# inferflow/inferflow

Hardware: AMD Instinct MI355X
Metric: decode tokens/sec, Llama-2-7B Q4 batch=1 greedy (whole job) (higher is better)
Workload: dtype i8 (Q8 activations x Q4_B32T1A weights, i32 dot, f32 scale, f16 I/O); 1 GPU; llama2_7b decode, Q4_B32T1A weights + F16 lm_head, F16 KV cache, batch 1 greedy, 16-token prompt, context 21..1851; parallelism=single, weights_bytes=4309647360

## Files before the change

include/inferflow_amd.h:

```cpp
#ifndef INFERFLOW_AMD_H_
#define INFERFLOW_AMD_H_

#include <stddef.h>
#include <stdint.h>

#ifdef __cplusplus
extern "C" {
#endif

typedef enum {
    IFA_F32 = 0, IFA_F16 = 1,
    IFA_Q8_B32T1 = 7, IFA_Q8_B32T2 = 8, IFA_Q6_B64T1 = 9, IFA_Q5_B64T1 = 10, IFA_Q5_B32T1 = 11,
    IFA_Q4_B16 = 12, IFA_Q4_B32T1A = 13, IFA_Q4_B32T1B = 14, IFA_Q4_B64T1 = 17, IFA_Q3H_B64T1 = 18,
    IFA_Q3_B32T1A = 19, IFA_Q3_B32T1B = 20, IFA_Q2_B32T1A = 21, IFA_Q2_B32T1B = 22
} ifa_dtype;

enum {
    IFA_OK = 0,
    IFA_ERR_ARG = -1,
    IFA_ERR_DTYPE = -2,
    IFA_ERR_HIP = -3,
    IFA_ERR_STATE = -4,
    IFA_ERR_NOMEM = -5
};
// ... 124 lines not shown
int ifa_model_create(const ifa_model_config *cfg, ifa_model **out);
int ifa_model_destroy(ifa_model *m);
int ifa_model_set_tensor(ifa_model *m, int layer, int tensor_id, int expert, int dtype,
                         const void *dev_src, size_t rows, size_t cols);
int ifa_model_set_tensor_f16(ifa_model *m, int layer, int tensor_id, int expert, int target_dtype,
                             const void *dev_src_f16, size_t rows, size_t cols);
int ifa_model_finalize(ifa_model *m);
int ifa_model_reset(ifa_model *m);
int ifa_model_kv_slots(ifa_model *m, int n_slots);
int ifa_model_select_kv(ifa_model *m, int slot);
int ifa_model_kv_copy(ifa_model *m, int src_slot, int dst_slot, int n_rows);
int ifa_model_kv_shift(ifa_model *m, int slot, int keep, int discard, int n_rows);
int ifa_kv_shift_rows(int kv_dtype, void *kcache, void *vcache, size_t kv_heads, size_t head_dim, int rope_order, int rope_cols,
                      const float *table_dev, size_t keep, size_t discard, size_t n_rows, ifa_stream stream);
int ifa_model_set_option(ifa_model *m, const char *name, int value);
int ifa_model_set_excluded_tokens(ifa_model *m, const int *ids_host, int n);
int ifa_model_perf_stat(ifa_model *m, int *keys_out, float *ms_out, int cap, int *n_out, int clear);
int ifa_model_fused_supported(ifa_model *m, char *why, size_t why_len);
int ifa_model_forward(ifa_model *m, const int *tokens_host, int n_tokens, int prefix_len,
                      void *logits_out_dev, int *next_token_host);
int ifa_model_decode(ifa_model *m, int first_token, int start_pos, int n_steps,
                     int *out_tokens_host, float *elapsed_ms);
int ifa_model_decode_prepare(ifa_model *m, int start_pos, int n_steps);
int ifa_model_decode_batch(ifa_model *m, int n, const int *tokens_host, const int *positions_host, const int *kv_slots_host,
                           int *next_tokens_host, void *logits_out_dev);
int ifa_model_decode_draft(ifa_model *m, int n, const int *tokens_host, int pos0, int *next_tokens_host, void *logits_out_dev);
int ifa_model_set_pool_excluded(ifa_model *m, const int *ids_host, int n);
int ifa_model_decode_pool(ifa_model *m, int token, int pos, int k, int *next_token_host,
                          int *pool_ids_host, unsigned short *pool_vals_host, int *pool_count_host);
int ifa_model_decode_batch_pool(ifa_model *m, int n, const int *tokens_host, const int *positions_host, const int *kv_slots_host,
                                int *next_tokens_host, int k, const int *rows_sel_host, int n_sel,
                                int *pool_ids_host, unsigned short *pool_vals_host, int *pool_counts_host);
int ifa_model_forward_pool(ifa_model *m, const int *tokens_host, int n_tokens, int prefix_len, void *logits_out_dev, int k,
                           int *next_token_host, int *pool_ids_host, unsigned short *pool_vals_host, int *pool_count_host);
int ifa_model_pool_lse(ifa_model *m, float *lse_host, int cap, int *n_out);
#define IFA_LOGIT_BIAS_MAX 1024
int ifa_model_logit_state_reset(ifa_model *m, int kv_slot, const int *prompt_host, int n_prompt, float rep, float freq, float pres,
                                const int *bias_ids_host, const float *bias_vals_host, int n_bias);
int ifa_model_logit_state_add(ifa_model *m, int n, const int *kv_slots_host, const int *tokens_host);
int ifa_model_pool_adjust(ifa_model *m, int n_sel, const int *state_slots_host);
int ifa_model_forward_score(ifa_model *m, const int *tokens_host, int n_tokens, int prefix_len, const int *targets_host,
                            float *lse_host, float *target_logit_host, int *next_token_host);
int ifa_model_get_buffer(ifa_model *m, const char *name, int layer, void **dptr, size_t *bytes);
void *ifa_model_stream(ifa_model *m);
int ifa_debug_alloc_fail_at(long long nth);
int ifa_debug_live_allocs(long long *count, long long *bytes);
// ... 59 lines not shown
```

inferflow_amd/_capi.py:

```python
import ctypes as C
import os

_HERE = os.path.dirname(os.path.abspath(__file__))
_LIB_PATH = os.environ.get("IFA_LIB") or os.path.join(_HERE, "lib", "libinferflow_amd.so")
_lib = None


class IfaError(RuntimeError):
    def __init__(self, code, msg):
        super().__init__("inferflow_amd error %d: %s" % (code, msg))
        self.code = code


def library_path():
    return _LIB_PATH


def lib():
    global _lib
    if _lib is None:
        if not os.path.exists(_LIB_PATH):
            raise ImportError(
                "inferflow_amd: %s is missing -- run `python __graft_entry__.py build` "
                "(hipcc --offload-arch=gfx950); there is no CPU fallback" % _LIB_PATH)
# ... 63 lines not shown
    "ifa_argmax": (_i, [_vp, _sz, _vp, _vp]),
    "ifa_argmax_masked": (_i, [_vp, _sz, _vp, _vp, _vp]),
    "ifa_topk_pool": (_i, [_vp, _sz, _sz, _i, _vp, _vp, _vp, _vp, _vp]),
    "ifa_logsumexp_workspace": (_sz, [_sz, _sz]),
    "ifa_logsumexp_rows": (_i, [_vp, _sz, _vp, _sz, _sz, _vp, _vp, _vp, _vp, _vp]),
    "ifa_logit_adjust_rows": (_i, [_vp, _sz, _vp, _vp, _sz, _sz, _vp, _vp, _vp, _vp, _vp]),
    "ifa_logit_state_reset": (_i, [_i, _vp, _sz, _f, _f, _f, _vp, _vp, _sz, _sz, _vp, _vp, _vp, _vp]),
    "ifa_logit_state_add": (_i, [_vp, _vp, _sz, _sz, _sz, _vp, _vp]),
    "ifa_model_create": (_i, [_vp, C.POINTER(_vp)]),
    "ifa_model_destroy": (_i, [_vp]),
    "ifa_debug_alloc_fail_at": (_i, [C.c_longlong]),
    "ifa_debug_live_allocs": (_i, [C.POINTER(C.c_longlong), C.POINTER(C.c_longlong)]),
    "ifa_model_set_tensor": (_i, [_vp, _i, _i, _i, _i, _vp, _sz, _sz]),
    "ifa_model_set_tensor_f16": (_i, [_vp, _i, _i, _i, _i, _vp, _sz, _sz]),
    "ifa_model_finalize": (_i, [_vp]),
    "ifa_model_reset": (_i, [_vp]),
    "ifa_model_set_option": (_i, [_vp, C.c_char_p, _i]),
    "ifa_model_set_excluded_tokens": (_i, [_vp, _vp, _i]),
    "ifa_model_perf_stat": (_i, [_vp, _vp, _vp, _i, _vp, _i]),
    "ifa_model_fused_supported": (_i, [_vp, C.c_char_p, _sz]),
    "ifa_model_forward": (_i, [_vp, _vp, _i, _i, _vp, _vp]),
    "ifa_model_decode": (_i, [_vp, _i, _i, _i, _vp, _vp]),
    "ifa_model_decode_prepare": (_i, [_vp, _i, _i]),
    "ifa_add_by_row_index": (_i, [_vp, _vp, _sz, _sz, _vp, _vp, _vp]),
    "ifa_model_kv_slots": (_i, [_vp, _i]),
    "ifa_model_select_kv": (_i, [_vp, _i]),
    "ifa_model_kv_copy": (_i, [_vp, _i, _i, _i]),
    "ifa_model_kv_shift": (_i, [_vp, _i, _i, _i, _i]),
    "ifa_kv_shift_rows": (_i, [_i, _vp, _vp, _sz, _sz, _i, _i, _vp, _sz, _sz, _sz, _vp]),
    "ifa_model_decode_batch": (_i, [_vp, _i, _vp, _vp, _vp, _vp, _vp]),
    "ifa_model_decode_draft": (_i, [_vp, _i, _vp, _i, _vp, _vp]),
    "ifa_model_set_pool_excluded": (_i, [_vp, _vp, _i]),
    "ifa_model_decode_pool": (_i, [_vp, _i, _i, _i, _vp, _vp, _vp, _vp]),
    "ifa_model_decode_batch_pool": (_i, [_vp, _i, _vp, _vp, _vp, _vp, _i, _vp, _i, _vp, _vp, _vp]),
    "ifa_model_forward_pool": (_i, [_vp, _vp, _i, _i, _vp, _i, _vp, _vp, _vp, _vp]),
    "ifa_model_pool_lse": (_i, [_vp, _vp, _i, _vp]),
    "ifa_model_logit_state_reset": (_i, [_vp, _i, _vp, _i, _f, _f, _f, _vp, _vp, _i]),
    "ifa_model_logit_state_add": (_i, [_vp, _i, _vp, _vp]),
    "ifa_model_pool_adjust": (_i, [_vp, _i, _vp]),
    "ifa_model_forward_score": (_i, [_vp, _vp, _i, _i, _vp, _vp, _vp, _vp]),
    "ifa_model_get_buffer": (_i, [_vp, C.c_char_p, _i, C.POINTER(_vp), C.POINTER(_sz)]),
    "ifa_model_stream": (_vp, [_vp]),
    "ifa_model_time_kernel": (_i, [_vp, _i, _i, _vp]),
    "ifa_model_set_stream": (_i, [_vp, _vp]),
    "ifa_model_tp_begin": (_i, [_vp, _i, _i]),
    "ifa_model_tp_begin_hidden": (_i, [_vp, _vp, _i]),
# ... 120 lines not shown
```

inferflow_amd/csrc/ifa_engine.hip:

```cpp
#include <mutex>
#include <unordered_map>
#include "ifa_engine_state.h"

namespace ifa {

namespace {
struct SpaceBook {
    std::mutex mu;
    std::unordered_map<void *, size_t> live;
    long long live_bytes = 0, fail_at = 0;
};
SpaceBook &book() { static SpaceBook *b = new SpaceBook(); return *b; }

template <class Alloc> int space_alloc(const char *call, void **p, size_t bytes, Alloc alloc)
{
    SpaceBook &b = book();
    *p = nullptr;
    {
        std::lock_guard<std::mutex> g(b.mu);
        if (b.fail_at > 0 && --b.fail_at == 0)
            return ifa_fail(IFA_ERR_HIP, "%s(%zu bytes) failed: out of memory (simulated: ifa_debug_alloc_fail_at)", call, bytes);
    }
    const hipError_t e = alloc(p, bytes);
    if (e != hipSuccess) {
// ... 61 lines not shown
{
    if (idx < 0 || idx >= (int)m->perf_spans.size()) return;
    if (hipEventRecord(m->perf_spans[(size_t)idx].e1, m->stream) != hipSuccess) (void)hipGetLastError();
}

int perf_collect(ifa_model *m)
{
    if (m->perf_spans.empty()) return IFA_OK;
    IFA_HIP_CHECK(hipStreamSynchronize(m->stream));
    for (auto &r : m->perf_spans) {
        float ms = 0.0f;
        if (hipEventElapsedTime(&ms, r.e0, r.e1) == hipSuccess) m->perf_map[r.key] += ms;
        else (void)hipGetLastError();
        m->perf_pool.push_back(r.e0); m->perf_pool.push_back(r.e1);
    }
    m->perf_spans.clear();
    return IFA_OK;
}

void drop_graphs(ifa_model *m)
{
    if (m->tp_graph_exec) { (void)hipGraphExecDestroy(m->tp_graph_exec); m->tp_graph_exec = nullptr; }
    if (m->tp_graph) { (void)hipGraphDestroy(m->tp_graph); m->tp_graph = nullptr; }
    if (m->graph_exec) { (void)hipGraphExecDestroy(m->graph_exec); m->graph_exec = nullptr; }
    if (m->graph) { (void)hipGraphDestroy(m->graph); m->graph = nullptr; }
    if (m->graph_exec_n) { (void)hipGraphExecDestroy(m->graph_exec_n); m->graph_exec_n = nullptr; }
    if (m->graph_n) { (void)hipGraphDestroy(m->graph_n); m->graph_n = nullptr; }
    for (auto &sl : m->slots) {
        if (sl.exec) { (void)hipGraphExecDestroy(sl.exec); sl.exec = nullptr; }
        if (sl.graph) { (void)hipGraphDestroy(sl.graph); sl.graph = nullptr; }
    }
    for (auto &kv : m->batch_graphs) if (kv.second) (void)hipGraphExecDestroy(kv.second);
    m->batch_graphs.clear();
    for (auto &kv : m->draft_graphs) if (kv.second) (void)hipGraphExecDestroy(kv.second);
    m->draft_graphs.clear();
}

int ensure_scratch(ifa_model *m, int T)
{
    if (T <= m->scratch_tokens) return IFA_OK;
    const ifa_model_config &c = m->cfg;
    const size_t D = c.dim, QD = (size_t)c.heads * c.head_dim, KVD = (size_t)c.kv_heads * c.head_dim, F = c.ffn;
    size_t maxcols = std::max(std::max(D, QD), F);
    Scratch n;
    int rc;
    if ((rc = n.x.alloc(T * D)) || (rc = n.x2.alloc(T * D)) || (rc = n.xn.alloc(T * D)) || (rc = n.hn.alloc(T * D)) || (rc = n.pn.alloc(T * D))
        || (rc = n.q.alloc(T * QD)) || (rc = n.k.alloc(T * KVD)) || (rc = n.v.alloc(T * KVD)) || (rc = n.att.alloc(T * QD))
        || (rc = n.a.alloc(T * D)) || (rc = n.f.alloc(T * D)) || (rc = n.t1.alloc(std::max<size_t>(T, 3) * F)) || (rc = n.t2.alloc(T * F))
        || (rc = n.logits.alloc((size_t)T * c.vocab)))
        return rc;
    if (!m->dqkv && (rc = n.dqkv.alloc(QD + 2 * KVD))) return rc;
    if (T <= 32 && !m->bqkv && ((rc = n.bqkv.alloc(32 * (QD + 2 * KVD))) || (rc = n.brope.alloc(32 * (size_t)c.head_dim)))) return rc;
    if (c.experts > 0) {
        const size_t cap = (size_t)T * (size_t)std::max(1, c.moe_top_k);
// ... 342 lines not shown
            int rc;
            if ((rc = k.alloc(bytes)) || (rc = v.alloc(bytes))) return rc;
            IFA_HIP_CHECK(hipMemsetAsync(k, 0, bytes, m->stream));
            IFA_HIP_CHECK(hipMemsetAsync(v, 0, bytes, m->stream));
            sl.k.push_back(std::move(k)); sl.v.push_back(std::move(v));
        }
        m->slots.push_back(std::move(sl));
    }
    IFA_HIP_CHECK(hipStreamSynchronize(m->stream));
    return IFA_OK;
}

int ifa_model_select_kv(ifa_model *m, int slot)
{
    IFA_REQUIRE(m && m->finalized, "ifa_model_select_kv: model not finalized");
    if (m->slots.empty()) m->slots.resize(1);
    IFA_REQUIRE(slot >= 0 && slot < (int)m->slots.size(), "ifa_model_select_kv: slot %d of %zu", slot, m->slots.size());
    if (slot == m->cur_slot) return IFA_OK;
    if (m->tp_graph_exec) { (void)hipGraphExecDestroy(m->tp_graph_exec); m->tp_graph_exec = nullptr; }
    if (m->tp_graph) { (void)hipGraphDestroy(m->tp_graph); m->tp_graph = nullptr; }
    ifa_model::KvSlot &out = m->slots[(size_t)m->cur_slot], &in = m->slots[(size_t)slot];
    out.k.clear(); out.v.clear();
    for (Layer &L : m->layers) { out.k.push_back(std::move(L.kcache)); out.v.push_back(std::move(L.vcache)); }
    out.graph = m->graph; out.exec = m->graph_exec;
    if (m->graph_exec_n) { (void)hipGraphExecDestroy(m->graph_exec_n); m->graph_exec_n = nullptr; }
    if (m->graph_n) { (void)hipGraphDestroy(m->graph_n); m->graph_n = nullptr; }
    for (size_t l = 0; l < m->layers.size(); l++) { m->layers[l].kcache = std::move(in.k[l]); m->layers[l].vcache = std::move(in.v[l]); }
    m->graph = in.graph; m->graph_exec = in.exec;
    in.k.clear(); in.v.clear(); in.graph = nullptr; in.exec = nullptr;
    m->cur_slot = slot;
    return IFA_OK;
}

int ifa_model_set_option(ifa_model *m, const char *name, int value)
{
    IFA_REQUIRE(m && name, "ifa_model_set_option: null pointer");
    if (strcmp(name, "pool_lse") == 0) { m->opt_pool_lse = value != 0; return IFA_OK; }
    struct { const char *n; int *p; } opts[] = {
        {"fused", &m->opt_fused}, {"graph", &m->opt_graph}, {"rpw_qkv", &m->opt_rpw_qkv}, {"rpw_wo", &m->opt_rpw_wo},
        {"rpw_ffn", &m->opt_rpw_ffn}, {"rpw_w2", &m->opt_rpw_w2}, {"rpw_lm", &m->opt_rpw_lm}, {"trace", &m->opt_trace},
        {"bench_mode", &m->opt_bench_mode}, {"touch_stride", &m->opt_touch_stride}, {"attn_split_ctx", &m->opt_attn_split_ctx}, {"batch_graph", &m->opt_batch_graph}, {"gemm_rows", &m->opt_gemm_rows}, {"batch_fused", &m->opt_batch_fused}, {"rows_mo", &m->opt_rows_mo}, {"debug_mo_alloc_fail", &m->opt_debug_mo_alloc_fail}, {"rows_kparts", &m->opt_rows_kparts}, {"prefill_chunk", &m->opt_prefill_chunk}, {"prefill_big_min", &m->opt_prefill_big_min}, {"prefill_mid", &m->opt_prefill_mid}, {"prefill_mid_max", &m->opt_prefill_mid_max}, {"prefill_res_mid", &m->opt_prefill_res_mid}, {"gemm_splitk", &m->opt_gemm_splitk}, {"moe_singles", &m->opt_moe_singles}, {"moe_overlap", &m->opt_moe_overlap}, {"prefill_big", &m->opt_prefill_big}, {"moe_router_fused", &m->opt_moe_router_fused}, {"tp_fuse_add", &m->opt_tp_fuse_add}, {"attn_q8", &m->opt_attn_q8}, {"attn_kt", &m->opt_attn_kt}, {"fuse_attn", &m->opt_fuse_attn}, {"fuse_ffn", &m->opt_fuse_ffn}, {"attn_post_as_residual", &m->opt_attn_post_as_residual}, {"chain_late_w2", &m->opt_chain_late_w2}, {"exact_order", &m->opt_exact_order}, {"perf_stat", &m->opt_perf_stat}, {"attn_nsplits", &m->opt_attn_nsplits}, {"attn_unload", &m->opt_attn_unload}, {"q3h_native", &m->opt_q3h_native}, {"fuse_attn_timeout_us", &m->opt_fuse_attn_timeout_us}, {"step_tail", &m->opt_step_tail}, {"graph_steps", &m->opt_graph_steps}, {"moe_device", &m->opt_moe_device}, 
        
        {"debug_layers", &m->opt_debug_layers}, {"debug_layer0", &m->opt_debug_layer0}, {"debug_hidden_in", &m->opt_debug_hidden_in}};
    for (auto &o : opts)
        if (strcmp(o.n, name) == 0) {
            *o.p = value;
            drop_graphs(m);
            return IFA_OK;
        }
    return ifa_fail(IFA_ERR_ARG, "ifa_model_set_option: unknown option '%s'", name);
}

int ifa_model_perf_stat(ifa_model *m, int *keys_out, float *ms_out, int cap, int *n_out, int clear)
{
    IFA_REQUIRE(m && n_out && cap >= 0 && (cap == 0 || (keys_out && ms_out)), "ifa_model_perf_stat: null pointer");
    IFA_HIP_CHECK(hipSetDevice(m->cfg.device));
    int rc = perf_collect(m);
    if (rc) return rc;
    int n = 0;
    for (auto &kv : m->perf_map) {
        if (n < cap) { keys_out[n] = kv.first; ms_out[n] = kv.second; }
        n++;
    }
    *n_out = n;
// ... 98 lines not shown
```

inferflow_amd/csrc/ifa_engine_decode.hip:

```cpp
#include "ifa_engine_state.h"

namespace ifae {

bool qkv_attn_layer_ok(const ifa_model *m, int l, int *gk_out);

static int attn_split_threshold(const ifa_model *m)
{
    if (m->opt_attn_split_ctx >= 0) return m->opt_attn_split_ctx;
    const ifa_model_config &c = m->cfg;
    bool tail = m->opt_attn_unload && m->opt_fuse_attn && waits_enabled() && dec_attn_smem(c.head_dim, c.max_ctx, 256) <= IFA_LDS_LIMIT;
    int gk = 0;
    for (int l = 0; tail && l < c.layers; l++) if (!qkv_attn_layer_ok(m, l, &gk)) tail = false;
    if (tail && (long long)c.kv_heads * gk > (long long)visible_cus()) tail = false;
    if (!tail) return 320;
    return c.heads > c.kv_heads ? 640 : 512;
}

void choose_attn_split(ifa_model *m, int reach)
{
    const int thr = attn_split_threshold(m);
    const int want = (thr > 0 && reach > thr) ? (reach > 8192 ? 16 : 8) : 0;
    if (want != m->attn_split) { m->attn_split = want; drop_graphs(m); }
    const int pb = reach <= 64 ? 64 : (reach <= 128 ? 128 : 256);
    if (pb != m->attn_pb) { m->attn_pb = pb; drop_graphs(m); }
}

__global__ void __launch_bounds__(256) k_touch(const uint8_t *__restrict__ p, size_t bytes, size_t stride, int *sink)
{
    size_t i = ((size_t)blockIdx.x * blockDim.x + threadIdx.x) * stride;
    int acc = 0;
    for (; i < bytes; i += (size_t)gridDim.x * blockDim.x * stride) acc += *reinterpret_cast<const int *>(p + i);
    if (acc == 0x7FFFFFFF) *sink = acc;
}

static long long *g_trace_ptr = nullptr;

bool fused_ok(const Tensor &t, bool long_rows)
{
    if (!t.present()) return false;
    if (fused_int8(t.dtype)) return t.tiled && (long_rows ? dec_gemv_supported_long(t.dtype, t.cols) : dec_gemv_supported(t.dtype, t.cols));
    return dec_gemv_h_supported(t.dtype, t.cols) && (long_rows || t.cols <= 8192);
}

template <int EPI, int NORM>
static int launch_dec_gemv(int w_dtype, const DecGemvParams &P, int wgs_per_cu_opt, hipStream_t s)
{
    if (!fused_int8(w_dtype) && w_dtype != Q3H_NATIVE) {
// ... 605 lines not shown
        std::swap(x, xnext);
    }
    if (m->st_on) return launch_lm_tail(m, x);
    if ((rc = launch_lm(m, x))) return rc;
    k_dec_argmax_advance<<<dim3(1), dim3(1024), 0, s>>>(m->logits, (int)m->g[T_LM_HEAD].rows, m->state, ifa_model::RING);
    IFA_LAUNCH_CHECK();
    return IFA_OK;
}

}

extern "C" {

int ifa_model_decode(ifa_model *m, int first_token, int start_pos, int n_steps, int *out_tokens_host, float *elapsed_ms)
{
    return decode_impl(m, first_token, start_pos, n_steps, out_tokens_host, elapsed_ms, false);
}

int ifa_model_decode_prepare(ifa_model *m, int start_pos, int n_steps)
{
    return decode_impl(m, 0, start_pos, n_steps, nullptr, nullptr, true);
}

}

namespace ifae {

int decode_impl(ifa_model *m, int first_token, int start_pos, int n_steps, int *out_tokens_host, float *elapsed_ms, bool prepare_only)
{
    IFA_REQUIRE(m && m->finalized, "ifa_model_decode: model not finalized");
    IFA_REQUIRE(n_steps > 0 && n_steps <= ifa_model::RING, "ifa_model_decode: n_steps %d (max %d per call)", n_steps, ifa_model::RING);
    IFA_REQUIRE(start_pos >= 0 && start_pos + n_steps <= m->cfg.max_ctx, "ifa_model_decode: positions [%d,%d) exceed max_ctx %d",
                start_pos, start_pos + n_steps, m->cfg.max_ctx);
    IFA_REQUIRE(m->g[T_EMBD].present() && m->g[T_LM_HEAD].present(), "ifa_model_decode: embeddings / lm_head missing (pipeline stage worker)");
    IFA_HIP_CHECK(hipSetDevice(m->cfg.device));
    std::string why;
    if (m->opt_exact_order) {
        if (prepare_only) return IFA_OK;
        int tok = first_token;
        for (int i = 0; i < n_steps; i++) {
            int nt = 0;
            int rc = forward_exact(m, tok, start_pos + i, nullptr, &nt);
            if (rc) return rc;
            if (out_tokens_host) out_tokens_host[i] = nt;
            tok = nt;
        }
        if (elapsed_ms) *elapsed_ms = -1.0f;
        return IFA_OK;
    }
// ... 9 lines not shown
        }
        if (elapsed_ms) *elapsed_ms = -1.0f;
        return IFA_OK;
    }
    static const bool trace_host = getenv("IFA_TRACE_DECODE") != nullptr;
    const auto th0 = std::chrono::steady_clock::now();
    auto th = [&](const char *what) {
        if (trace_host) fprintf(stderr, "decode-host %-28s %8.1f us\n", what, std::chrono::duration<double, std::micro>(std::chrono::steady_clock::now() - th0).count());
    };
    int rc = ensure_scratch(m, 1);
    if (rc) return rc;
    if (m->opt_q3h_native && (rc = ensure_q3hn(m))) return rc;
    hipStream_t s = m->stream;
    choose_attn_split(m, start_pos + n_steps);
    if ((rc = qkv_attn_ready(m))) return rc;
    if ((rc = step_tail_ready(m))) return rc;
    m->host_pinned[0] = first_token; m->host_pinned[1] = start_pos; m->host_pinned[2] = 0;
    IFA_HIP_CHECK(hipMemcpyAsync(m->state, m->host_pinned, 3 * sizeof(int), hipMemcpyHostToDevice, s));
    if (m->qa_on || m->ch_on) {
        m->qa_calls = (m->qa_calls % 4000u) + 1u;
        m->host_pinned[6] = (int)m->qa_calls;
        IFA_HIP_CHECK(hipMemcpyAsync(m->qa_call, m->host_pinned + 6, sizeof(int), hipMemcpyHostToDevice, s));
    }
    if (m->opt_graph && !m->graph_exec) {
        IFA_HIP_CHECK(hipStreamSynchronize(s));
        IFA_HIP_CHECK(hipStreamBeginCapture(s, hipStreamCaptureModeThreadLocal));
        rc = enqueue_fused_step(m);
        hipGraph_t gph = nullptr;
        hipError_t e = hipStreamEndCapture(s, &gph);
        if (rc) { if (gph) (void)hipGraphDestroy(gph); return rc; }
        if (e != hipSuccess) return ifa_fail(IFA_ERR_HIP, "hipStreamEndCapture: %s", hipGetErrorString(e));
        if (m->graph) (void)hipGraphDestroy(m->graph);
        m->graph = gph;
        IFA_HIP_CHECK(hipGraphInstantiate(&m->graph_exec, m->graph, nullptr, nullptr, 0));
    }
    const int S = m->opt_graph_steps;
    if (m->opt_graph && S > 1 && n_steps >= S && (!m->graph_exec_n || m->graph_n_steps != S)) {
        if (m->graph_exec_n) { (void)hipGraphExecDestroy(m->graph_exec_n); m->graph_exec_n = nullptr; }
        if (m->graph_n) { (void)hipGraphDestroy(m->graph_n); m->graph_n = nullptr; }
        IFA_HIP_CHECK(hipStreamSynchronize(s));
        IFA_HIP_CHECK(hipStreamBeginCapture(s, hipStreamCaptureModeThreadLocal));
        for (int i = 0; i < S && !rc; i++) rc = enqueue_fused_step(m);
        hipGraph_t gph = nullptr;
        hipError_t e = hipStreamEndCapture(s, &gph);
        if (rc) { if (gph) (void)hipGraphDestroy(gph); return rc; }
        if (e != hipSuccess) return ifa_fail(IFA_ERR_HIP, "hipStreamEndCapture: %s", hipGetErrorString(e));
        m->graph_n = gph; m->graph_n_steps = S;
        IFA_HIP_CHECK(hipGraphInstantiate(&m->graph_exec_n, m->graph_n, nullptr, nullptr, 0));
    }
    if (prepare_only) return IFA_OK;
    th("state copies enqueued");
    hipEvent_t e0 = nullptr, e1 = nullptr;
    if (elapsed_ms) { IFA_HIP_CHECK(hipEventCreate(&e0)); IFA_HIP_CHECK(hipEventCreate(&e1)); IFA_HIP_CHECK(hipEventRecord(e0, s)); }
    th("events created, first recorded");
    if (m->st_on && (rc = launch_gather(m))) return rc;
    for (int i = 0; i < n_steps;) {
        if (m->opt_graph && m->graph_exec_n && m->graph_n_steps == S && S > 1 && n_steps - i >= S) { IFA_HIP_CHECK(hipGraphLaunch(m->graph_exec_n, s)); i += S; continue; }
        if (m->opt_graph) IFA_HIP_CHECK(hipGraphLaunch(m->graph_exec, s));
        else if ((rc = enqueue_fused_step(m))) return rc;
        i++;
    }
    th("steps enqueued");
    if (elapsed_ms) IFA_HIP_CHECK(hipEventRecord(e1, s));
    if ((rc = pool_enqueue(m, m->logits, 1))) return rc;
    IFA_HIP_CHECK(hipMemcpyAsync(m->host_pinned + 8, m->state + 8, sizeof(int) * (size_t)n_steps, hipMemcpyDeviceToHost, s));
    int *qerr = m->host_pinned + 8 + ifa_model::RING;
    qerr[0] = 0;
    if (m->qa_on || m->ch_on) IFA_HIP_CHECK(hipMemcpyAsync(qerr, m->qa_err, 4, hipMemcpyDeviceToHost, s));
    th("copies back enqueued");
    IFA_HIP_CHECK(hipStreamSynchronize(s));
    th("stream synchronised");
    if (qerr[0] != 0) {
        (void)hipMemsetAsync(m->qa_err, 0, 16, s);
        (void)hipStreamSynchronize(s);
        if (elapsed_ms) { (void)hipEventDestroy(e0); (void)hipEventDestroy(e1); }
        m->opt_fuse_attn = 0; m->opt_fuse_ffn = 0;
        drop_graphs(m);
        waits_disable("the fused QKV + attention launch timed out waiting for sibling workgroups");
        return ifa_fail(IFA_ERR_STATE, "fused decode launch: a wait for another workgroup's rows timed out (code 0x%x: 0x5_ q | k | v / attention output, 0x6_ Wo output, 0x9_ chained FFN launch); "
                        "the results of this call are not valid -- repeat it: options fuse_attn / fuse_ffn are off now (five-launch step)", (unsigned)qerr[0]);
    }
    if (elapsed_ms) { IFA_HIP_CHECK(hipEventElapsedTime(elapsed_ms, e0, e1)); (void)hipEventDestroy(e0); (void)hipEventDestroy(e1); }
    if (out_tokens_host) memcpy(out_tokens_host, m->host_pinned + 8, sizeof(int) * (size_t)n_steps);
// ... 74 lines not shown
```

inferflow_amd/csrc/ifa_engine_state.h:

```cpp
#pragma once
#include <chrono>
#include <cstdlib>
#include <cstring>
#include <map>
#include <string>
#include <vector>
#include "ifa_host.h"
#include "ifa_buf_hip.h"
#include "ifa_decode_kernels.h"
#include "ifa_decode_attn.h"
#include "ifa_decode_gemv.h"
#include "ifa_moe.h"
#include "ifa_gemm_rows_mfma.h"
#include "ifa_gemm_big.h"
#include "ifa_decode_lmhead_tail.h"
#include "ifa_decode_singles.h"
#include "ifa_decode_qkv_attn.h"
#include "ifa_decode_chain.h"

using namespace ifa;

namespace ifae {


enum { T_EMBD = 0, T_OUT_NORM = 1, T_OUT_NORM_B = 2, T_LM_HEAD = 3,
       T_ATTN_NORM = 10, T_ATTN_NORM_B = 11, T_WQ = 12, T_WK = 13, T_WV = 14, T_WO = 15,
       T_FFN_NORM = 16, T_FFN_NORM_B = 17, T_W1 = 18, T_W2 = 19, T_W3 = 20, T_MOE_GATE = 21,
       T_WQ_B = 22, T_WK_B = 23, T_WV_B = 24, T_WO_B = 25, T_W1_B = 26, T_W2_B = 27, T_W3_B = 28,
       T_ATTN_POST_NORM = 29, T_ATTN_POST_NORM_B = 30, T_FFN_POST_NORM = 31, T_FFN_POST_NORM_B = 32,
       T_MAX = 36 };

struct Tensor {
    int dtype = -1;
    DevBuf<void> data;
    DevBuf<void> tiled;
    DevBuf<void> mo;
    DevBuf<void> q3hn;
    DevBuf<void> x32;
    size_t rows = 0, cols = 0;
    bool present() const { return data != nullptr; }
};
// ... 27 lines not shown
    DevBuf<half_t> pn;
};


}
using namespace ifae;

struct ifa_model : Scratch {
    ifa_model_config cfg;
    std::vector<Layer> layers;
    Tensor g[10];
    hipStream_t stream = nullptr;
    hipStream_t side_stream = nullptr; Event ev_fork, ev_join; int opt_moe_overlap = 1;
    bool own_stream = true;
    bool finalized = false;
    int opt_moe_device = 1;
    DevBuf<int> state;
    DevBuf<float> rope_tab;
    DevBuf<long long> trace;
    int opt_trace = 0, opt_bench_mode = 0, opt_touch_stride = 65536;
    PinBuf<int> host_pinned;
    int scratch_tokens = 0;
    size_t kv_row_bytes = 0;
    hipGraph_t graph = nullptr;
    hipGraphExec_t graph_exec = nullptr;
    hipGraph_t graph_n = nullptr; hipGraphExec_t graph_exec_n = nullptr; int graph_n_steps = 0, opt_graph_steps = 1;
    struct PendingAdd { const half_t *x = nullptr, *add = nullptr, *bias = nullptr; half_t *out = nullptr; bool on = false; } pend;
    int opt_tp_fuse_add = 1;
    DevPin<void> batch_tab;
    std::map<int, hipGraphExec_t> batch_graphs;
    std::map<int, hipGraphExec_t> draft_graphs;
    DecAttnSplitWs attn_ws = {nullptr, nullptr, nullptr, 8};
    DevBuf<half_t> attn_ws_S; DevBuf<float> attn_ws_lmax, attn_ws_opart;
    int opt_attn_unload = 1;
    int opt_attn_nsplits = 0;
    int opt_fuse_attn = 1, opt_fuse_attn_timeout_us = 20000, qa_on = 0, qa_gk = 0;
    DevBuf<unsigned long long> qa_gran;
    DevBuf<unsigned> qa_call, qa_err; unsigned qa_calls = 0;
    int opt_fuse_ffn = 0, ch_on = 0, opt_chain_late_w2 = 0;
    int opt_q3h_native = 0;
    int opt_perf_stat = 0;
    struct PerfSpanRec { int key; hipEvent_t e0, e1; };
    std::vector<PerfSpanRec> perf_spans;
    std::vector<hipEvent_t> perf_pool;
    std::map<int, float> perf_map;
    int opt_exact_order = 0;
    DevBuf<float> exact_rope_tab;
    DevBuf<uint32_t> ch_gran, ch_flags;
    int opt_step_tail = 1, st_on = 0;
    DevBuf<unsigned long long> st_keys; DevBuf<unsigned> st_counter;
    int attn_pb = 256, opt_attn_kt = 1;
    int attn_split = 0, opt_attn_split_ctx = -1, opt_batch_graph = 0, opt_gemm_rows = 1, opt_batch_fused = 1, opt_moe_router_fused = 1, opt_prefill_big = 1, opt_rows_mo = 1, opt_moe_singles = 1;
    struct KvSlot { std::vector<DevBuf<void>> k, v; hipGraph_t graph = nullptr; hipGraphExec_t exec = nullptr; };
    std::vector<KvSlot> slots;
    int cur_slot = 0;
    int opt_attn_q8 = 1;
    DevBuf<half_t> tp_a, tp_f, tp_hid, tp_logits;
    DevBuf<float> tp_best, tp_gather;
    DevBuf<int> tp_tok;
    hipGraph_t tp_graph = nullptr;
    hipGraphExec_t tp_graph_exec = nullptr;
    struct TpKey {
        unsigned long long tp = 0, world = 0; int tp_size = 0, stage = 0, n_stages = 0, prev = 0, next = 0, src = 0, voff = 0, force = 0, fuse = 0, slot = 0, oneshot = 0;
        bool operator==(const TpKey &o) const { return tp == o.tp && world == o.world && tp_size == o.tp_size && stage == o.stage && n_stages == o.n_stages
                && prev == o.prev && next == o.next && src == o.src && voff == o.voff && force == o.force && fuse == o.fuse && slot == o.slot
                && oneshot == o.oneshot; }
    } tp_key;
    const ifa_tp_topology *topo = nullptr;
    int opt_attn_post_as_residual = 1;
    int opt_fused = 1, opt_graph = 1, opt_rpw_qkv = 0, opt_rpw_wo = 0, opt_rpw_ffn = 0, opt_rpw_w2 = 0, opt_rpw_lm = 0;
    int opt_debug_layers = 0;
    int opt_debug_layer0 = 0, opt_debug_hidden_in = 0;
    int opt_prefill_big_min = 47;
    int opt_prefill_chunk = 1;
    int opt_prefill_mid = 1, opt_prefill_mid_max = 768;
    int opt_prefill_res_mid = 2048;
    int opt_rows_kparts = 1, opt_gemm_splitk = 1;
    int opt_debug_mo_alloc_fail = 0;
    struct PoolReq {
        int k = 0;
        int n_sel = 0;
        const int *rows_sel = nullptr;
        int chunk0 = 0; bool last_chunk = true;
        int done = 0;
        bool lse = false;
        std::vector<int> adj;
    } pool;
    DevBuf<unsigned> pool_excl;
    DevPin<void> pool_blk;
// ... 174 lines not shown
```

inferflow_amd/csrc/ifa_engine_tp.hip:

```cpp
#include "ifa_engine_state.h"

namespace ifae {

__global__ void __launch_bounds__(1024) k_tp_local_best(const half_t *__restrict__ v_all, size_t row_stride, int n, int vocab_offset,
                                                        const int *__restrict__ excl, float *__restrict__ best_all)
{
    __shared__ float bv[16];
    __shared__ int bi[16];
    const half_t *v = v_all + (size_t)blockIdx.x * row_stride;
    float *best_out = best_all + 2 * (size_t)blockIdx.x;
    const int ne = excl ? min(max(excl[0], 0), 3) : 0;
    const int e0 = ne > 0 ? excl[1] : -1, e1 = ne > 1 ? excl[2] : -1, e2 = ne > 2 ? excl[3] : -1;
    float best = -INFINITY; int besti = 0x7FFFFFFF;
    argmax_scan(v, (size_t)n, e0, e1, e2, (int)threadIdx.x, (int)blockDim.x, best, besti, vocab_offset);
#pragma unroll
    for (int mk = 32; mk > 0; mk >>= 1) {
        const float ob = __shfl_xor(best, mk); const int oi = __shfl_xor(besti, mk);
        if (ob > best || (ob == best && oi < besti)) { best = ob; besti = oi; }
    }
    const int wave = threadIdx.x >> 6, lane = threadIdx.x & 63;
    if (lane == 0) { bv[wave] = best; bi[wave] = besti; }
    __syncthreads();
    if (threadIdx.x == 0) {
        for (int w = 1; w < (int)(blockDim.x >> 6); w++)
// ... 365 lines not shown
{
    IFA_REQUIRE(n >= 1 && n <= ifa_model::RING && tokens_host && positions_host && kv_slots_host, "ifa_model_tp_decode_batch: bad arguments");
    int rc = tp_check(m, topo, "ifa_model_tp_decode_batch");
    if (rc) return rc;
    m->topo = topo;
    rc = forward_batch(m, n, tokens_host, positions_host, kv_slots_host, next_tokens_host, logits_shard_out_dev);
    m->topo = nullptr;
    if (rc == IFA_OK) { (void)hipStreamSynchronize(m->stream); rc = tp_oneshot_status(m, *topo, "ifa_model_tp_decode_batch"); }
    return rc;
}

int ifa_model_tp_decode(ifa_model *m, const ifa_tp_topology *topo, int first_token, int start_pos, int n_steps,
                        int *out_tokens_host, float *elapsed_ms)
{
    IFA_REQUIRE(out_tokens_host, "ifa_model_tp_decode: null pointer");
    IFA_REQUIRE(n_steps >= 1 && n_steps <= ifa_model::RING, "ifa_model_tp_decode: n_steps %d (1..%d)", n_steps, ifa_model::RING);
    int rc = tp_check(m, topo, "ifa_model_tp_decode");
    if (rc) return rc;
    IFA_REQUIRE(start_pos >= 0 && start_pos + n_steps <= m->cfg.max_ctx, "ifa_model_tp_decode: positions %d..%d exceed max_ctx %d",
                start_pos, start_pos + n_steps, m->cfg.max_ctx);
    const ifa_tp_topology &t = *topo;
    hipStream_t s = m->stream;
    choose_attn_split(m, start_pos + n_steps);
    m->host_pinned[0] = first_token; m->host_pinned[1] = start_pos; m->host_pinned[2] = 0;
    IFA_HIP_CHECK(hipMemcpyAsync(m->state, m->host_pinned, 3 * sizeof(int), hipMemcpyHostToDevice, s));
    const bool use_graph = m->opt_graph && t.n_stages == 1 && (!t.tp || ifa_comm_capturable(t.tp));
    {
        ifa_model::TpKey key;
        key.tp = ifa_comm_serial(t.tp); key.world = ifa_comm_serial(t.world); key.tp_size = t.tp ? ifa_comm_size(t.tp) : 1;
        key.stage = t.stage; key.n_stages = t.n_stages; key.prev = t.prev_rank; key.next = t.next_rank; key.src = t.token_src;
        key.voff = t.vocab_offset; key.force = t.force_collectives; key.fuse = m->opt_tp_fuse_add; key.slot = m->cur_slot;
        key.oneshot = t.tp ? ifa_comm_oneshot(t.tp) : 0;
        if (m->tp_graph_exec && !(key == m->tp_key)) {
            (void)hipGraphExecDestroy(m->tp_graph_exec); m->tp_graph_exec = nullptr;
            if (m->tp_graph) { (void)hipGraphDestroy(m->tp_graph); m->tp_graph = nullptr; }
        }
        m->tp_key = key;
    }
    int done = 0;
    if (!(use_graph && m->tp_graph_exec)) {
        if ((rc = tp_step(m, t, first_token, start_pos))) return rc;
        done = 1;
        if (use_graph && done < n_steps) {
            IFA_HIP_CHECK(hipStreamSynchronize(s));
            IFA_HIP_CHECK(hipStreamBeginCapture(s, hipStreamCaptureModeThreadLocal));
            rc = tp_step(m, t, -1, -1);
            hipGraph_t gph = nullptr;
            hipError_t e = hipStreamEndCapture(s, &gph);
            if (rc || e != hipSuccess) {
                if (gph) (void)hipGraphDestroy(gph);
                (void)hipGetLastError();
                m->tp_graph_exec = nullptr;
            } else {
                m->tp_graph = gph;
                if (hipGraphInstantiate(&m->tp_graph_exec, gph, nullptr, nullptr, 0) != hipSuccess) { m->tp_graph_exec = nullptr; (void)hipGetLastError(); }
// ... 24 lines not shown
```

inferflow_amd/worker.py:

```python
import ctypes as C

import numpy as np

from . import _capi, dtypes as dt
from ._capi import ModelConfig, check, lib

T_EMBD, T_OUT_NORM, T_OUT_NORM_B, T_LM_HEAD = 0, 1, 2, 3
T_ATTN_NORM, T_ATTN_NORM_B, T_WQ, T_WK, T_WV, T_WO = 10, 11, 12, 13, 14, 15
T_FFN_NORM, T_FFN_NORM_B, T_W1, T_W2, T_W3, T_MOE_GATE = 16, 17, 18, 19, 20, 21
T_WQ_B, T_WK_B, T_WV_B, T_WO_B, T_W1_B, T_W2_B, T_W3_B = 22, 23, 24, 25, 26, 27, 28
T_ATTN_POST_NORM, T_ATTN_POST_NORM_B, T_FFN_POST_NORM, T_FFN_POST_NORM_B = 29, 30, 31, 32

_DEFAULTS = dict(norm_kind=0, act_kind=0, is_glu=1, rope_order=2, use_alibi=0, parallel_attn=0, share_input=0,
                 rope_theta=10000.0, partial_rotary=1.0, kq_scale=1.0, eps=1e-5, kv_dtype=dt.F16,
                 full_quant_gemv=1, experts=0, moe_top_k=0, moe_norm_topk=1, tp_rank=0, tp_size=1, device=0,
                 attn_norm_base=0.0, ffn_norm_base=0.0, out_norm_base=0.0, attn_out_scale=1.0, ffn_out_scale=1.0, out_scale=1.0,
                 embd_scale=0.0)


class DecodeWorker:
    def __init__(self, **kw):
        cfg = ModelConfig()
        vals = dict(_DEFAULTS)
        vals.update(kw)
# ... 161 lines not shown

    def logit_state_add(self, kv_slots, tokens):
        sl = np.ascontiguousarray(kv_slots, np.int32).reshape(-1)
        tk = np.ascontiguousarray(tokens, np.int32).reshape(-1)
        assert sl.size == tk.size
        check(lib().ifa_model_logit_state_add(self._h, sl.size, sl.ctypes.data_as(C.c_void_p), tk.ctypes.data_as(C.c_void_p)))

    def pool_adjust(self, state_slots):
        sl = np.ascontiguousarray(state_slots, np.int32).reshape(-1)
        check(lib().ifa_model_pool_adjust(self._h, sl.size, sl.ctypes.data_as(C.c_void_p) if sl.size else None))

    def forward_score(self, tokens, prefix_len, targets):
        toks = np.ascontiguousarray(tokens, np.int32)
        tg = np.ascontiguousarray(targets, np.int32).reshape(-1)
        assert tg.size == toks.size, (tg.size, toks.size)
        lse, tl = np.zeros(toks.size, np.float32), np.zeros(toks.size, np.float32)
        nxt = C.c_int(-1)
        check(lib().ifa_model_forward_score(self._h, toks.ctypes.data_as(C.c_void_p), toks.size, int(prefix_len), tg.ctypes.data_as(C.c_void_p),
                                            lse.ctypes.data_as(C.c_void_p), tl.ctypes.data_as(C.c_void_p), C.byref(nxt)))
        return nxt.value, lse, tl

    def decode_prepare(self, start_pos, n_steps):
        check(lib().ifa_model_decode_prepare(self._h, int(start_pos), int(n_steps)))

    def time_kernel(self, which, iters=200):
        us = C.c_float(0)
        check(lib().ifa_model_time_kernel(self._h, which, iters, C.byref(us)))
        return us.value

    def get_tensor_host(self, layer, tid):
        d, p, r, c = C.c_int(), C.c_void_p(), C.c_size_t(), C.c_size_t()
        rc = lib().ifa_model_get_tensor(self._h, layer, tid, C.byref(d), C.byref(p), C.byref(r), C.byref(c))
        if rc == 1:
            return None
        check(rc)
        nbytes = r.value * dt.row_bytes(d.value, c.value)
        out = np.empty(nbytes, np.uint8)
        check(lib().ifa_memcpy_d2h(out.ctypes.data_as(C.c_void_p), p, nbytes, None))
        check(lib().ifa_stream_sync(None))
        if d.value == dt.F16:
            out = out.view(np.uint16)
        return d.value, out, r.value, c.value

    def get_expert_tensor_host(self, layer, expert, tid):
        d, p, r, c = C.c_int(), C.c_void_p(), C.c_size_t(), C.c_size_t()
        rc = lib().ifa_model_get_expert_tensor(self._h, layer, expert, tid, C.byref(d), C.byref(p), C.byref(r), C.byref(c))
# ... 250 lines not shown
```

Before: 624.0 tokens/s.

## Bucket decode steps by context length with per-bucket cached step graphs

```diff
diff --git a/include/inferflow_amd.h b/include/inferflow_amd.h
--- a/include/inferflow_amd.h
+++ b/include/inferflow_amd.h
@@ -170,6 +170,8 @@
 int ifa_model_decode(ifa_model *m, int first_token, int start_pos, int n_steps,
                      int *out_tokens_host, float *elapsed_ms);
 int ifa_model_decode_prepare(ifa_model *m, int start_pos, int n_steps);
+int ifa_model_step_captures(ifa_model *m, long long *n);
+int ifa_step_bucket_runs(int start_pos, int n_steps, int step_buckets, int edge_lo, int edge_hi, int *out9, int *n_runs);
 int ifa_model_decode_batch(ifa_model *m, int n, const int *tokens_host, const int *positions_host, const int *kv_slots_host,
                            int *next_tokens_host, void *logits_out_dev);
 int ifa_model_decode_draft(ifa_model *m, int n, const int *tokens_host, int pos0, int *next_tokens_host, void *logits_out_dev);
diff --git a/inferflow_amd/_capi.py b/inferflow_amd/_capi.py
--- a/inferflow_amd/_capi.py
+++ b/inferflow_amd/_capi.py
@@ -109,6 +109,8 @@
     "ifa_model_forward": (_i, [_vp, _vp, _i, _i, _vp, _vp]),
     "ifa_model_decode": (_i, [_vp, _i, _i, _i, _vp, _vp]),
     "ifa_model_decode_prepare": (_i, [_vp, _i, _i]),
+    "ifa_model_step_captures": (_i, [_vp, C.POINTER(C.c_longlong)]),
+    "ifa_step_bucket_runs": (_i, [_i, _i, _i, _i, _i, C.POINTER(_i), C.POINTER(_i)]),
     "ifa_add_by_row_index": (_i, [_vp, _vp, _sz, _sz, _vp, _vp, _vp]),
     "ifa_model_kv_slots": (_i, [_vp, _i]),
     "ifa_model_select_kv": (_i, [_vp, _i]),
diff --git a/inferflow_amd/csrc/ifa_engine.hip b/inferflow_amd/csrc/ifa_engine.hip
--- a/inferflow_amd/csrc/ifa_engine.hip
+++ b/inferflow_amd/csrc/ifa_engine.hip
@@ -107,14 +107,15 @@
 {
     if (m->tp_graph_exec) { (void)hipGraphExecDestroy(m->tp_graph_exec); m->tp_graph_exec = nullptr; }
     if (m->tp_graph) { (void)hipGraphDestroy(m->tp_graph); m->tp_graph = nullptr; }
-    if (m->graph_exec) { (void)hipGraphExecDestroy(m->graph_exec); m->graph_exec = nullptr; }
-    if (m->graph) { (void)hipGraphDestroy(m->graph); m->graph = nullptr; }
-    if (m->graph_exec_n) { (void)hipGraphExecDestroy(m->graph_exec_n); m->graph_exec_n = nullptr; }
-    if (m->graph_n) { (void)hipGraphDestroy(m->graph_n); m->graph_n = nullptr; }
-    for (auto &sl : m->slots) {
-        if (sl.exec) { (void)hipGraphExecDestroy(sl.exec); sl.exec = nullptr; }
-        if (sl.graph) { (void)hipGraphDestroy(sl.graph); sl.graph = nullptr; }
-    }
+    auto drop = [](std::vector<ifa_model::StepGraph> &tab) {
+        for (auto &g : tab) {
+            if (g.exec) (void)hipGraphExecDestroy(g.exec);
+            if (g.graph) (void)hipGraphDestroy(g.graph);
+        }
+        tab.clear();
+    };
+    drop(m->step_graphs);
+    for (auto &sl : m->slots) drop(sl.graphs);
     for (auto &kv : m->batch_graphs) if (kv.second) (void)hipGraphExecDestroy(kv.second);
     m->batch_graphs.clear();
     for (auto &kv : m->draft_graphs) if (kv.second) (void)hipGraphExecDestroy(kv.second);
@@ -503,12 +504,10 @@
     ifa_model::KvSlot &out = m->slots[(size_t)m->cur_slot], &in = m->slots[(size_t)slot];
     out.k.clear(); out.v.clear();
     for (Layer &L : m->layers) { out.k.push_back(std::move(L.kcache)); out.v.push_back(std::move(L.vcache)); }
-    out.graph = m->graph; out.exec = m->graph_exec;
-    if (m->graph_exec_n) { (void)hipGraphExecDestroy(m->graph_exec_n); m->graph_exec_n = nullptr; }
-    if (m->graph_n) { (void)hipGraphDestroy(m->graph_n); m->graph_n = nullptr; }
+    out.graphs = std::move(m->step_graphs);
     for (size_t l = 0; l < m->layers.size(); l++) { m->layers[l].kcache = std::move(in.k[l]); m->layers[l].vcache = std::move(in.v[l]); }
-    m->graph = in.graph; m->graph_exec = in.exec;
-    in.k.clear(); in.v.clear(); in.graph = nullptr; in.exec = nullptr;
+    m->step_graphs = std::move(in.graphs);
+    in.k.clear(); in.v.clear(); in.graphs.clear();
     m->cur_slot = slot;
     return IFA_OK;
 }
@@ -520,7 +519,7 @@
     struct { const char *n; int *p; } opts[] = {
         {"fused", &m->opt_fused}, {"graph", &m->opt_graph}, {"rpw_qkv", &m->opt_rpw_qkv}, {"rpw_wo", &m->opt_rpw_wo},
         {"rpw_ffn", &m->opt_rpw_ffn}, {"rpw_w2", &m->opt_rpw_w2}, {"rpw_lm", &m->opt_rpw_lm}, {"trace", &m->opt_trace},
-        {"bench_mode", &m->opt_bench_mode}, {"touch_stride", &m->opt_touch_stride}, {"attn_split_ctx", &m->opt_attn_split_ctx}, {"batch_graph", &m->opt_batch_graph}, {"gemm_rows", &m->opt_gemm_rows}, {"batch_fused", &m->opt_batch_fused}, {"rows_mo", &m->opt_rows_mo}, {"debug_mo_alloc_fail", &m->opt_debug_mo_alloc_fail}, {"rows_kparts", &m->opt_rows_kparts}, {"prefill_chunk", &m->opt_prefill_chunk}, {"prefill_big_min", &m->opt_prefill_big_min}, {"prefill_mid", &m->opt_prefill_mid}, {"prefill_mid_max", &m->opt_prefill_mid_max}, {"prefill_res_mid", &m->opt_prefill_res_mid}, {"gemm_splitk", &m->opt_gemm_splitk}, {"moe_singles", &m->opt_moe_singles}, {"moe_overlap", &m->opt_moe_overlap}, {"prefill_big", &m->opt_prefill_big}, {"moe_router_fused", &m->opt_moe_router_fused}, {"tp_fuse_add", &m->opt_tp_fuse_add}, {"attn_q8", &m->opt_attn_q8}, {"attn_kt", &m->opt_attn_kt}, {"fuse_attn", &m->opt_fuse_attn}, {"fuse_ffn", &m->opt_fuse_ffn}, {"attn_post_as_residual", &m->opt_attn_post_as_residual}, {"chain_late_w2", &m->opt_chain_late_w2}, {"exact_order", &m->opt_exact_order}, {"perf_stat", &m->opt_perf_stat}, {"attn_nsplits", &m->opt_attn_nsplits}, {"attn_unload", &m->opt_attn_unload}, {"q3h_native", &m->opt_q3h_native}, {"fuse_attn_timeout_us", &m->opt_fuse_attn_timeout_us}, {"step_tail", &m->opt_step_tail}, {"graph_steps", &m->opt_graph_steps}, {"moe_device", &m->opt_moe_device}, 
+        {"bench_mode", &m->opt_bench_mode}, {"touch_stride", &m->opt_touch_stride}, {"attn_split_ctx", &m->opt_attn_split_ctx}, {"batch_graph", &m->opt_batch_graph}, {"gemm_rows", &m->opt_gemm_rows}, {"batch_fused", &m->opt_batch_fused}, {"rows_mo", &m->opt_rows_mo}, {"debug_mo_alloc_fail", &m->opt_debug_mo_alloc_fail}, {"rows_kparts", &m->opt_rows_kparts}, {"prefill_chunk", &m->opt_prefill_chunk}, {"prefill_big_min", &m->opt_prefill_big_min}, {"prefill_mid", &m->opt_prefill_mid}, {"prefill_mid_max", &m->opt_prefill_mid_max}, {"prefill_res_mid", &m->opt_prefill_res_mid}, {"gemm_splitk", &m->opt_gemm_splitk}, {"moe_singles", &m->opt_moe_singles}, {"moe_overlap", &m->opt_moe_overlap}, {"prefill_big", &m->opt_prefill_big}, {"moe_router_fused", &m->opt_moe_router_fused}, {"tp_fuse_add", &m->opt_tp_fuse_add}, {"attn_q8", &m->opt_attn_q8}, {"attn_kt", &m->opt_attn_kt}, {"fuse_attn", &m->opt_fuse_attn}, {"fuse_ffn", &m->opt_fuse_ffn}, {"attn_post_as_residual", &m->opt_attn_post_as_residual}, {"chain_late_w2", &m->opt_chain_late_w2}, {"exact_order", &m->opt_exact_order}, {"perf_stat", &m->opt_perf_stat}, {"attn_nsplits", &m->opt_attn_nsplits}, {"attn_unload", &m->opt_attn_unload}, {"q3h_native", &m->opt_q3h_native}, {"fuse_attn_timeout_us", &m->opt_fuse_attn_timeout_us}, {"step_tail", &m->opt_step_tail}, {"graph_steps", &m->opt_graph_steps}, {"moe_device", &m->opt_moe_device}, {"step_buckets", &m->opt_step_buckets}, {"attn_pb_force", &m->opt_attn_pb_force},
         
         {"debug_layers", &m->opt_debug_layers}, {"debug_layer0", &m->opt_debug_layer0}, {"debug_hidden_in", &m->opt_debug_hidden_in}};
     for (auto &o : opts)
diff --git a/inferflow_amd/csrc/ifa_engine_decode.hip b/inferflow_amd/csrc/ifa_engine_decode.hip
--- a/inferflow_amd/csrc/ifa_engine_decode.hip
+++ b/inferflow_amd/csrc/ifa_engine_decode.hip
@@ -21,8 +21,6 @@
     const int thr = attn_split_threshold(m);
     const int want = (thr > 0 && reach > thr) ? (reach > 8192 ? 16 : 8) : 0;
     if (want != m->attn_split) { m->attn_split = want; drop_graphs(m); }
-    const int pb = reach <= 64 ? 64 : (reach <= 128 ? 128 : 256);
-    if (pb != m->attn_pb) { m->attn_pb = pb; drop_graphs(m); }
 }
 
 __global__ void __launch_bounds__(256) k_touch(const uint8_t *__restrict__ p, size_t bytes, size_t stride, int *sink)
@@ -674,9 +672,49 @@
     return decode_impl(m, 0, start_pos, n_steps, nullptr, nullptr, true);
 }
 
+int ifa_model_step_captures(ifa_model *m, long long *n)
+{
+    IFA_REQUIRE(m && n, "ifa_model_step_captures: null pointer");
+    *n = m->step_captures;
+    return IFA_OK;
+}
+
+int ifa_step_bucket_runs(int start_pos, int n_steps, int step_buckets, int edge_lo, int edge_hi, int *out9, int *n_runs)
+{
+    IFA_REQUIRE(out9 && n_runs, "ifa_step_bucket_runs: null pointer");
+    StepRun runs[3];
+    const int n = step_bucket_runs(start_pos, n_steps, step_buckets, edge_lo > 0 ? edge_lo : STEP_EDGE_LO, edge_hi > 0 ? edge_hi : STEP_EDGE_HI, runs);
+    IFA_REQUIRE(n > 0, "ifa_step_bucket_runs: start_pos %d, n_steps %d, edges %d / %d", start_pos, n_steps, edge_lo, edge_hi);
+    for (int i = 0; i < n; i++) { out9[3 * i] = runs[i].first; out9[3 * i + 1] = runs[i].n; out9[3 * i + 2] = runs[i].pb; }
+    *n_runs = n;
+    return IFA_OK;
+}
+
 }
 
 namespace ifae {
+
+static int step_graph(ifa_model *m, int n, hipGraphExec_t *exec)
+{
+    for (const ifa_model::StepGraph &g : m->step_graphs)
+        if (g.split == m->attn_split && g.pb == m->attn_pb && g.n == n) { *exec = g.exec; return IFA_OK; }
+    hipStream_t s = m->stream;
+    IFA_HIP_CHECK(hipStreamSynchronize(s));
+    IFA_HIP_CHECK(hipStreamBeginCapture(s, hipStreamCaptureModeThreadLocal));
+    int rc = IFA_OK;
+    for (int i = 0; i < n && !rc; i++) rc = enqueue_fused_step(m);
+    ifa_model::StepGraph g;
+    g.split = m->attn_split; g.pb = m->attn_pb; g.n = n;
+    hipError_t e = hipStreamEndCapture(s, &g.graph);
+    if (rc) { if (g.graph) (void)hipGraphDestroy(g.graph); return rc; }
+    if (e != hipSuccess) return ifa_fail(IFA_ERR_HIP, "hipStreamEndCapture: %s", hipGetErrorString(e));
+    e = hipGraphInstantiate(&g.exec, g.graph, nullptr, nullptr, 0);
+    if (e != hipSuccess) { (void)hipGraphDestroy(g.graph); return ifa_fail(IFA_ERR_HIP, "hipGraphInstantiate: %s", hipGetErrorString(e)); }
+    m->step_graphs.push_back(g);
+    m->step_captures++;
+    *exec = g.exec;
+    return IFA_OK;
+}
 
 int decode_impl(ifa_model *m, int first_token, int start_pos, int n_steps, int *out_tokens_host, float *elapsed_ms, bool prepare_only)
 {
@@ -732,43 +770,32 @@
         m->host_pinned[6] = (int)m->qa_calls;
         IFA_HIP_CHECK(hipMemcpyAsync(m->qa_call, m->host_pinned + 6, sizeof(int), hipMemcpyHostToDevice, s));
     }
-    if (m->opt_graph && !m->graph_exec) {
-        IFA_HIP_CHECK(hipStreamSynchronize(s));
-        IFA_HIP_CHECK(hipStreamBeginCapture(s, hipStreamCaptureModeThreadLocal));
-        rc = enqueue_fused_step(m);
-        hipGraph_t gph = nullptr;
-        hipError_t e = hipStreamEndCapture(s, &gph);
-        if (rc) { if (gph) (void)hipGraphDestroy(gph); return rc; }
-        if (e != hipSuccess) return ifa_fail(IFA_ERR_HIP, "hipStreamEndCapture: %s", hipGetErrorString(e));
-        if (m->graph) (void)hipGraphDestroy(m->graph);
-        m->graph = gph;
-        IFA_HIP_CHECK(hipGraphInstantiate(&m->graph_exec, m->graph, nullptr, nullptr, 0));
-    }
+    StepRun runs[3];
+    int n_runs;
+    if (m->opt_attn_pb_force == 64 || m->opt_attn_pb_force == 128 || m->opt_attn_pb_force == 256) { runs[0] = {0, n_steps, m->opt_attn_pb_force}; n_runs = 1; }
+    else n_runs = step_bucket_runs(start_pos, n_steps, m->opt_step_buckets && !m->attn_split, STEP_EDGE_LO, STEP_EDGE_HI, runs);
     const int S = m->opt_graph_steps;
-    if (m->opt_graph && S > 1 && n_steps >= S && (!m->graph_exec_n || m->graph_n_steps != S)) {
-        if (m->graph_exec_n) { (void)hipGraphExecDestroy(m->graph_exec_n); m->graph_exec_n = nullptr; }
-        if (m->graph_n) { (void)hipGraphDestroy(m->graph_n); m->graph_n = nullptr; }
-        IFA_HIP_CHECK(hipStreamSynchronize(s));
-        IFA_HIP_CHECK(hipStreamBeginCapture(s, hipStreamCaptureModeThreadLocal));
-        for (int i = 0; i < S && !rc; i++) rc = enqueue_fused_step(m);
-        hipGraph_t gph = nullptr;
-        hipError_t e = hipStreamEndCapture(s, &gph);
-        if (rc) { if (gph) (void)hipGraphDestroy(gph); return rc; }
-        if (e != hipSuccess) return ifa_fail(IFA_ERR_HIP, "hipStreamEndCapture: %s", hipGetErrorString(e));
-        m->graph_n = gph; m->graph_n_steps = S;
-        IFA_HIP_CHECK(hipGraphInstantiate(&m->graph_exec_n, m->graph_n, nullptr, nullptr, 0));
-    }
+    hipGraphExec_t exec1[3] = {nullptr, nullptr, nullptr}, execS[3] = {nullptr, nullptr, nullptr};
+    for (int r = 0; r < n_runs && m->opt_graph; r++) {
+        m->attn_pb = runs[r].pb;
+        if ((rc = step_graph(m, 1, &exec1[r]))) return rc;
+        if (S > 1 && runs[r].n >= S && (rc = step_graph(m, S, &execS[r]))) return rc;
+    }
+    m->attn_pb = runs[n_runs - 1].pb;
     if (prepare_only) return IFA_OK;
     th("state copies enqueued");
     hipEvent_t e0 = nullptr, e1 = nullptr;
     if (elapsed_ms) { IFA_HIP_CHECK(hipEventCreate(&e0)); IFA_HIP_CHECK(hipEventCreate(&e1)); IFA_HIP_CHECK(hipEventRecord(e0, s)); }
     th("events created, first recorded");
     if (m->st_on && (rc = launch_gather(m))) return rc;
-    for (int i = 0; i < n_steps;) {
-        if (m->opt_graph && m->graph_exec_n && m->graph_n_steps == S && S > 1 && n_steps - i >= S) { IFA_HIP_CHECK(hipGraphLaunch(m->graph_exec_n, s)); i += S; continue; }
-        if (m->opt_graph) IFA_HIP_CHECK(hipGraphLaunch(m->graph_exec, s));
-        else if ((rc = enqueue_fused_step(m))) return rc;
-        i++;
+    for (int r = 0; r < n_runs; r++) {
+        m->attn_pb = runs[r].pb;
+        for (int i = 0; i < runs[r].n;) {
+            if (execS[r] && runs[r].n - i >= S) { IFA_HIP_CHECK(hipGraphLaunch(execS[r], s)); i += S; continue; }
+            if (m->opt_graph) IFA_HIP_CHECK(hipGraphLaunch(exec1[r], s));
+            else if ((rc = enqueue_fused_step(m))) return rc;
+            i++;
+        }
     }
     th("steps enqueued");
     if (elapsed_ms) IFA_HIP_CHECK(hipEventRecord(e1, s));
diff --git a/inferflow_amd/csrc/ifa_engine_state.h b/inferflow_amd/csrc/ifa_engine_state.h
--- a/inferflow_amd/csrc/ifa_engine_state.h
+++ b/inferflow_amd/csrc/ifa_engine_state.h
@@ -17,6 +17,7 @@
 #include "ifa_decode_singles.h"
 #include "ifa_decode_qkv_attn.h"
 #include "ifa_decode_chain.h"
+#include "ifa_step_buckets.h"
 
 using namespace ifa;
 
@@ -90,9 +91,11 @@
     PinBuf<int> host_pinned;
     int scratch_tokens = 0;
     size_t kv_row_bytes = 0;
-    hipGraph_t graph = nullptr;
-    hipGraphExec_t graph_exec = nullptr;
-    hipGraph_t graph_n = nullptr; hipGraphExec_t graph_exec_n = nullptr; int graph_n_steps = 0, opt_graph_steps = 1;
+    struct StepGraph { int split = 0, pb = 0, n = 1; hipGraph_t graph = nullptr; hipGraphExec_t exec = nullptr; };
+    std::vector<StepGraph> step_graphs;
+    long long step_captures = 0;
+    int opt_graph_steps = 1;
+    int opt_step_buckets = 1, opt_attn_pb_force = 0;
     struct PendingAdd { const half_t *x = nullptr, *add = nullptr, *bias = nullptr; half_t *out = nullptr; bool on = false; } pend;
     int opt_tp_fuse_add = 1;
     DevPin<void> batch_tab;
@@ -119,7 +122,7 @@
     DevBuf<unsigned long long> st_keys; DevBuf<unsigned> st_counter;
     int attn_pb = 256, opt_attn_kt = 1;
     int attn_split = 0, opt_attn_split_ctx = -1, opt_batch_graph = 0, opt_gemm_rows = 1, opt_batch_fused = 1, opt_moe_router_fused = 1, opt_prefill_big = 1, opt_rows_mo = 1, opt_moe_singles = 1;
-    struct KvSlot { std::vector<DevBuf<void>> k, v; hipGraph_t graph = nullptr; hipGraphExec_t exec = nullptr; };
+    struct KvSlot { std::vector<DevBuf<void>> k, v; std::vector<StepGraph> graphs; };
     std::vector<KvSlot> slots;
     int cur_slot = 0;
     int opt_attn_q8 = 1;
@@ -129,10 +132,10 @@
     hipGraph_t tp_graph = nullptr;
     hipGraphExec_t tp_graph_exec = nullptr;
     struct TpKey {
-        unsigned long long tp = 0, world = 0; int tp_size = 0, stage = 0, n_stages = 0, prev = 0, next = 0, src = 0, voff = 0, force = 0, fuse = 0, slot = 0, oneshot = 0;
+        unsigned long long tp = 0, world = 0; int tp_size = 0, stage = 0, n_stages = 0, prev = 0, next = 0, src = 0, voff = 0, force = 0, fuse = 0, slot = 0, oneshot = 0, pb = 0;
         bool operator==(const TpKey &o) const { return tp == o.tp && world == o.world && tp_size == o.tp_size && stage == o.stage && n_stages == o.n_stages
                 && prev == o.prev && next == o.next && src == o.src && voff == o.voff && force == o.force && fuse == o.fuse && slot == o.slot
-                && oneshot == o.oneshot; }
+                && oneshot == o.oneshot && pb == o.pb; }
     } tp_key;
     const ifa_tp_topology *topo = nullptr;
     int opt_attn_post_as_residual = 1;
diff --git a/inferflow_amd/csrc/ifa_engine_tp.hip b/inferflow_amd/csrc/ifa_engine_tp.hip
--- a/inferflow_amd/csrc/ifa_engine_tp.hip
+++ b/inferflow_amd/csrc/ifa_engine_tp.hip
@@ -411,6 +411,7 @@
     const ifa_tp_topology &t = *topo;
     hipStream_t s = m->stream;
     choose_attn_split(m, start_pos + n_steps);
+    m->attn_pb = step_bucket(start_pos + n_steps);
     m->host_pinned[0] = first_token; m->host_pinned[1] = start_pos; m->host_pinned[2] = 0;
     IFA_HIP_CHECK(hipMemcpyAsync(m->state, m->host_pinned, 3 * sizeof(int), hipMemcpyHostToDevice, s));
     const bool use_graph = m->opt_graph && t.n_stages == 1 && (!t.tp || ifa_comm_capturable(t.tp));
@@ -419,7 +420,7 @@
         key.tp = ifa_comm_serial(t.tp); key.world = ifa_comm_serial(t.world); key.tp_size = t.tp ? ifa_comm_size(t.tp) : 1;
         key.stage = t.stage; key.n_stages = t.n_stages; key.prev = t.prev_rank; key.next = t.next_rank; key.src = t.token_src;
         key.voff = t.vocab_offset; key.force = t.force_collectives; key.fuse = m->opt_tp_fuse_add; key.slot = m->cur_slot;
-        key.oneshot = t.tp ? ifa_comm_oneshot(t.tp) : 0;
+        key.oneshot = t.tp ? ifa_comm_oneshot(t.tp) : 0; key.pb = m->attn_pb;
         if (m->tp_graph_exec && !(key == m->tp_key)) {
             (void)hipGraphExecDestroy(m->tp_graph_exec); m->tp_graph_exec = nullptr;
             if (m->tp_graph) { (void)hipGraphDestroy(m->tp_graph); m->tp_graph = nullptr; }
diff --git a/inferflow_amd/csrc/ifa_step_buckets.h b/inferflow_amd/csrc/ifa_step_buckets.h
--- /dev/null
+++ b/inferflow_amd/csrc/ifa_step_buckets.h
@@ -0,0 +1,28 @@
+#pragma once
+
+namespace ifae {
+
+static constexpr int STEP_EDGE_LO = 64, STEP_EDGE_HI = 128;
+
+struct StepRun { int first, n, pb; };
+
+static inline int step_bucket(int keys, int edge_lo = STEP_EDGE_LO, int edge_hi = STEP_EDGE_HI)
+{
+    return keys <= edge_lo ? 64 : (keys <= edge_hi ? 128 : 256);
+}
+
+static inline int step_bucket_runs(int start_pos, int n_steps, int per_step, int edge_lo, int edge_hi, StepRun out[3])
+{
+    if (n_steps < 1 || start_pos < 0 || edge_lo < 1 || edge_hi < edge_lo) return 0;
+    if (!per_step) { out[0] = {0, n_steps, step_bucket(start_pos + n_steps, edge_lo, edge_hi)}; return 1; }
+    const int ends[3] = {edge_lo - start_pos, edge_hi - start_pos, n_steps};
+    const int pbs[3] = {64, 128, 256};
+    int n = 0, first = 0;
+    for (int b = 0; b < 3; b++) {
+        const int end = ends[b] < first ? first : (ends[b] > n_steps ? n_steps : ends[b]);
+        if (end > first) { out[n++] = {first, end - first, pbs[b]}; first = end; }
+    }
+    return n;
+}
+
+}
diff --git a/inferflow_amd/worker.py b/inferflow_amd/worker.py
--- a/inferflow_amd/worker.py
+++ b/inferflow_amd/worker.py
@@ -207,6 +207,11 @@
 
     def decode_prepare(self, start_pos, n_steps):
         check(lib().ifa_model_decode_prepare(self._h, int(start_pos), int(n_steps)))
+
+    def step_captures(self):
+        n = C.c_longlong(0)
+        check(lib().ifa_model_step_captures(self._h, C.byref(n)))
+        return n.value
 
     def time_kernel(self, which, iters=200):
         us = C.c_float(0)
```

After: 623.4 tokens/s. No clear change (-0.1%).
